# talmolab/track-mjx

Hardware: AMD Instinct MI355X
Metric: env-steps/sec (whole node), rodent task @ 4096 envs/GPU (higher is better)
Workload: dtype f32

## Files before the change

### track_mjx_amd/csrc/wave_physics.h

```cpp
#pragma once
#include "tm_common.h"
#include "wave_layout.h"

#ifdef TM_HOST_EMU
#define TMW_NL 64
#define TMW_FOR for (int lane = 0; lane < 64; lane++)
#define TMW_SYNC() do { } while (0)
#define TMW_LI lane
#define TMW_LANE_DECL
#else
#define TMW_NL 1
#define TMW_FOR if (true)
#ifdef TMW_HARD_SYNC
#define TMW_SYNC() __syncthreads()
#else
#define TMW_SYNC() do { __builtin_amdgcn_fence(__ATOMIC_RELEASE, "wavefront"); __builtin_amdgcn_wave_barrier(); __builtin_amdgcn_fence(__ATOMIC_ACQUIRE, "wavefront"); } while (0)
#endif
#define TMW_LI 0
#define TMW_LANE_DECL const int lane = c.lane;
#endif
#define TMW_REG(type, name) type name[TMW_NL]
#ifdef TM_HOST_EMU
#define TMW_DUP_LANES_OK 0
#else
#define TMW_DUP_LANES_OK 1
#endif
#define TMW_DS 7

#ifdef TM_HOST_EMU
typedef const DModel TmwModel;
#else
typedef const __attribute__((address_space(4))) DModel TmwModel;
#endif
#define TMW_LOCAL(name, n, src) float name[n]; { _Pragma("unroll") for (int k_ = 0; k_ < (n); k_++) name[k_] = (src)[k_]; }
#ifdef TMW_RAND
#define TMW_RAND_ONLY(...) __VA_ARGS__
#define TMW_SCALE(x, s) tmw_scaled((x), c.s)
#ifdef TM_HOST_EMU
TM_DEV float tmw_scaled(float x, float s) { volatile float r = x * s; return r; }
#else
TM_DEV float tmw_scaled(float x, float s) { float r = x * s; asm volatile("" : "+v"(r)); return r; }
#endif
TM_DEV float tmw_rand_invweight(float t, float mu, float impratio) {
  const float mm = tmw_scaled(mu, mu), a = tmw_scaled(mm, t), b = tmw_scaled(t + a, 2.f), d = tmw_scaled(b, mu), e = tmw_scaled(d, mu);
  return e / impratio;
}
#define TMW_CON_IW(cc) tmw_rand_invweight(m.con_tw[cc], TMW_MU(cc), m.impratio)
#else
#define TMW_RAND_ONLY(...)
#define TMW_SCALE(x, s) x
#define TMW_CON_IW(cc) m.con_invweight[cc]
#endif
#define TMW_EMU_HAS_QA 1
struct WCtx {
  TmwModel *mp;
  float *L;
  float *st;
  int n, e;
  int lane;
  unsigned long long *prof;
  unsigned long long tlast;
  float *dump;
  int nact;
  int nla;
  int rs;
  unsigned kmask[TMW_NL];
  const float *action;
  float qfs0[TMW_NL], qfs1[TMW_NL];
  float dg0[TMW_NL], dg1[TMW_NL];
  float wp0[TMW_NL], wp1[TMW_NL];
  float qa0[TMW_NL], qa1[TMW_NL];
  float ma0[TMW_NL], ma1[TMW_NL];
  int tp0[TMW_NL], tp1[TMW_NL];
  float *mspill;
  TMW_RAND_ONLY(float s_f, s_a, s_d;)
};
#define TMW_STATS(K) L[(K).l_com + 3]
#if defined(TMW_PROFILE) && !defined(TM_HOST_EMU)
#define TMW_TICK(idx) do { unsigned long long t_ = __builtin_amdgcn_s_memtime(); if (c.prof && c.lane == 0) c.prof[idx] += t_ - c.tlast; c.tlast = t_; } while (0)
#define TMW_TICK2(idx) TMW_TICK(idx)
#define TMW_COUNT(idx, v) do { if (c.prof && c.lane == 0) c.prof[idx] += (v); } while (0)
#else
#define TMW_TICK(idx) do { } while (0)
#define TMW_TICK2(idx) do { } while (0)
#define TMW_COUNT(idx, v) do { } while (0)
#endif
#define WST(off, i) c.st[c.rs ? (size_t)c.e * (size_t)c.rs + (size_t)((off) + (i)) : (size_t)((off) + (i)) * (size_t)c.n + (size_t)c.e]

#define TMW_ACT(a) (*(K.lean ? &WST(m.s_act, (a)) : &L[K.l_act + (a)]))
#define TMW_QFS(i) (K.lean ? ((i) < 64 ? c.qfs0[TMW_LI] : c.qfs1[TMW_LI]) : L[K.l_qfrc_smooth + (i)])
#define TMW_QFS_SET(i, v) do { if (!K.lean) L[K.l_qfrc_smooth + (i)] = (v); else if ((i) < 64) c.qfs0[TMW_LI] = (v); else c.qfs1[TMW_LI] = (v); } while (0)
#ifdef TMW_NO_QA_REGS
#define TMW_QAREG(K) 0
#else
#define TMW_QAREG(K) ((K).lean)
#endif
#define TMW_QA(i) (TMW_QAREG(K) ? ((i) < 64 ? c.qa0[TMW_LI] : c.qa1[TMW_LI]) : L[K.l_qacc + (i)])
#define TMW_QA_SET(i, v) do { if (!TMW_QAREG(K)) L[K.l_qacc + (i)] = (v); else if ((i) < 64) c.qa0[TMW_LI] = (v); else c.qa1[TMW_LI] = (v); } while (0)
#define TMW_MA(i) (TMW_QAREG(K) ? ((i) < 64 ? c.ma0[TMW_LI] : c.ma1[TMW_LI]) : L[K.l_Ma + (i)])
#define TMW_MA_SET(i, v) do { if (!TMW_QAREG(K)) L[K.l_Ma + (i)] = (v); else if ((i) < 64) c.ma0[TMW_LI] = (v); else c.ma1[TMW_LI] = (v); } while (0)
#define TMW_OK1(K) (lane + 64 < (K).nv)
#define TMW_I1(K) (TMW_OK1(K) ? lane + 64 : lane)
#define TMW_MA1(K, i1) (TMW_QAREG(K) ? c.ma1[TMW_LI] : L[(K).l_Ma + (i1)])
#define TMW_QA1(K, i1) (TMW_QAREG(K) ? c.qa1[TMW_LI] : L[(K).l_qacc + (i1)])
#define TMW_DG(i) ((i) < 64 ? c.dg0[TMW_LI] : c.dg1[TMW_LI])
#define TMW_WP(i) ((i) < 64 ? c.wp0[TMW_LI] : c.wp1[TMW_LI])
#define TMW_WP_SET(i, v) do { if ((i) < 64) c.wp0[TMW_LI] = (v); else c.wp1[TMW_LI] = (v); } while (0)
#define TMW_MU(cc) (K.lean ? TMW_SCALE(m.con_mu[0], s_f) : L[K.l_con_mu + (cc)])
#ifdef TMW_NO_EFCD_PACK
#define TMW_DIDX(kr) (kr)
#else
#define TMW_DIDX(kr) (K.lean ? ((kr) < c.nla ? (kr) : c.nla + (((kr) - c.nla) >> 2)) : (kr))
#endif
#define TMW_LIMSIGN(K) ((signed char *)(L + (K).l_lim_sign))
TM_DEV int tm_f2i(float f) { int i; __builtin_memcpy(&i, &f, 4); return i; }
TM_DEV float tm_i2f(int i) { float f; __builtin_memcpy(&f, &i, 4); return f; }

#ifdef TM_HOST_EMU
TM_DEV float tmw_sum(const float *v) { float s = 0.f; for (int i = 0; i < 64; i++) s += v[i]; return s; }
TM_DEV float tmw_readlane(const float *v, int src) { return v[src]; }
#else
template <int CTRL, int ROW_MASK, int BANK_MASK>
TM_DEV float tmw_dpp_add(float v) {
  int moved = __builtin_amdgcn_update_dpp(0, tm_f2i(v), CTRL, ROW_MASK, BANK_MASK, false);
  return v + tm_i2f(moved);
}
#ifdef TMW_SHFL_REDUCE
TM_DEV float tmw_sum(const float *vp) {
  float v = vp[0];
  for (int off = 32; off >= 1; off >>= 1) v += __shfl_xor(v, off);
  return v;
}
TM_DEV float tmw_readlane(const float *v, int src) { return __shfl(v[0], src); }
#define tmw_sum_dpp tmw_sum_unused
#define tmw_readlane_dpp tmw_readlane_unused
#else
#define tmw_sum_dpp tmw_sum
#define tmw_readlane_dpp tmw_readlane
#endif
TM_DEV float tmw_sum_dpp(const float *vp) {
  float v = vp[0];
  v = tmw_dpp_add<0x111, 0xf, 0xf>(v);
  v = tmw_dpp_add<0x112, 0xf, 0xf>(v);
  v = tmw_dpp_add<0x114, 0xf, 0xf>(v);
  v = tmw_dpp_add<0x118, 0xf, 0xf>(v);
  v = tmw_dpp_add<0x142, 0xf, 0xf>(v);
  v = tmw_dpp_add<0x143, 0xf, 0xf>(v);
  return tm_i2f(__builtin_amdgcn_readlane(tm_f2i(v), 63));
}
TM_DEV float tmw_readlane_dpp(const float *v, int src) { return tm_i2f(__builtin_amdgcn_readlane(tm_f2i(v[0]), src)); }
#endif
#ifdef TM_HOST_EMU
template <int WIDTH> TM_DEV float tmw_sum_w(const float *v) { return tmw_sum(v); }
#else
template <int WIDTH> TM_DEV float tmw_sum_w(const float *vp) {
  float v = vp[0];
  v = tmw_dpp_add<0x111, 0xf, 0xf>(v);
  v = tmw_dpp_add<0x112, 0xf, 0xf>(v);
  v = tmw_dpp_add<0x114, 0xf, 0xf>(v);
  v = tmw_dpp_add<0x118, 0xf, 0xf>(v);
  if (WIDTH <= 16) return tm_i2f(__builtin_amdgcn_readlane(tm_f2i(v), 15));
  v = tmw_dpp_add<0x142, 0xf, 0xf>(v);
  if (WIDTH <= 32) return tm_i2f(__builtin_amdgcn_readlane(tm_f2i(v), 31));
  v = tmw_dpp_add<0x143, 0xf, 0xf>(v);
  return tm_i2f(__builtin_amdgcn_readlane(tm_f2i(v), 63));
}
#endif
#ifdef TM_HOST_EMU
TM_DEV int tmw_table2(const float *a0, const float *a1, int idx) { return tm_f2i(idx < 64 ? a0[idx] : a1[idx - 64]); }
#else
TM_DEV int tmw_table2(const float *a0, const float *a1, int idx) { return __builtin_amdgcn_readlane(tm_f2i(idx < 64 ? a0[0] : a1[0]), idx & 63); }
#endif

#ifdef TM_HOST_EMU
TM_DEV int tmw_prefix(const int *flag, int *excl) { int s = 0; for (int l = 0; l < 64; l++) { excl[l] = s; s += flag[l] != 0; } return s; }
#else
TM_DEV int tmw_prefix(const int *flag, int *excl) {
  unsigned long long b = __builtin_amdgcn_ballot_w64(flag[0] != 0);
  excl[0] = (int)__builtin_amdgcn_mbcnt_hi((unsigned)(b >> 32), __builtin_amdgcn_mbcnt_lo((unsigned)b, 0u));
  return __builtin_popcountll(b);
}
#endif
#define TMW_ROWMAP(K) ((unsigned char *)(L + (K).l_rowmap))
#define TMW_CCROW(K) ((unsigned char *)(L + (K).l_ccrow))
#define TMW_CONGRP(K) ((unsigned char *)(L + (K).l_con_grpb) + (K).ncon)

TM_DEV float tmw_load_state(WCtx &c, const WLayout &K, const float *action) {
  TmwModel &m = *c.mp; float *L = c.L; TMW_LANE_DECL
  TMW_FOR { for (int i = lane; i < K.lds_floats; i += 64) L[i] = 0.f; }
  TMW_SYNC();
  TMW_FOR {
    for (int i = lane; i < K.nq + K.nv + (K.lean ? 0 : K.nu); i += 64) L[K.l_qpos + i] = WST(m.s_qpos, i);
    if (K.lean) {
      c.tp0[TMW_LI] = m.tpack[lane < K.nv ? lane : 0]; c.tp1[TMW_LI] = m.tpack[lane + 64 < K.nv ? lane + 64 : 64];
      for (int g = lane; g < K.ngroup; g += 64) L[K.l_tgrp + g] = tm_i2f(m.gpack[g]);
    } else {
      for (int i = lane; i < 2 * K.nv; i += 64) {
        int dof = i >> 1, extra = (i & 1) ? m.dof_wsub[dof] + 1 : m.dof_limrow[dof] + 1;
        L[K.l_tdof + i] = tm_i2f(m.tdof[i] | (extra << 24));
      }
      for (int g = lane; g < K.ngroup; g += 64) ((signed char *)(L + K.l_tgrp))[g] = (signed char)m.grp_lastdof[g];
    }
    for (int cc = lane; cc < K.ncon; cc += 64) { if (!K.lean) L[K.l_con_mu + cc] = TMW_SCALE(m.con_mu[cc], s_f); TMW_CONGRP(K)[cc] = (unsigned char)m.con_grp[cc]; }
    {
      int su = lane / 6;
      bool ok = lane < m.n_wsub * 6;
      c.kmask[TMW_LI] = ok ? m.wsub_cmask[su][0] : 0u;
    }
  }
  TMW_SYNC();
  return WST(m.s_time, 0);
}
#define TMW_MEND(w0) ((w0) & 0xffff)
#define TMW_DEPTH(w0) (((w0) >> 16) & 0xff)
#define TMW_ADR(w0) (((w0) & 0xffff) - TMW_DEPTH(w0))
#define TMW_LIMROW1(w0) (((w0) >> 24) & 0xff)
#define TMW_WSUB1(w1) (((w1) >> 24) & 0xff)
#define TMW_W0(i) tm_f2i(L[K.l_tdof + 2 * (i)])
#define TMW_W1(i) tm_f2i(L[K.l_tdof + 2 * (i) + 1])
TM_DEV int tmw_anc(int i, int q, int w1) {
  int r = i - (w1 & 0xff);
  return q <= r ? i - q : ((w1 >> 8) & 0xff) + r - q;
}
#ifdef TM_HOST_EMU
TM_DEV int tmw_opaque_v(int x) { return x; }
#else
TM_DEV int tmw_opaque_v(int x) { asm volatile("" : "+v"(x)); return x; }
#endif
#define TMW_TP(i) tmw_opaque_v((i) < 64 ? c.tp0[TMW_LI] : c.tp1[TMW_LI])
#define TMW_TP_MEND(p) ((p) & 0x7ff)
#define TMW_TP_DEPTH(p) (((p) >> 11) & 0x3f)
#define TMW_TP_RUN(p) (((p) >> 17) & 0x1f)
#define TMW_TP_WSUB1(p) (((p) >> 22) & 0xf)
TM_DEV int tmw_anc_r(int i, int q, int r, int jp1) { return q <= r ? i - q : jp1 + r - q; }
TM_DEV void tmw_store_state(WCtx &c, const WLayout &K, float time) {
  TmwModel &m = *c.mp; float *L = c.L; TMW_LANE_DECL
  TMW_FOR {
    for (int i = lane; i < K.nq + K.nv + (K.lean ? 0 : K.nu); i += 64) WST(m.s_qpos, i) = L[K.l_qpos + i];
    if (lane == 0) WST(m.s_time, 0) = time;
  }
  TMW_SYNC();
}

TM_DEV void tmw_put_con_frame(float *L, const WLayout &K, int cc, const float *fr) {
  if (K.lean) { if (cc == 0) for (int k = 0; k < 3; k++) L[K.l_con_frame + k] = fr[k]; for (int k = 0; k < 3; k++) L[K.l_con_frame + 3 + cc * 3 + k] = fr[3 + k]; }
  else for (int k = 0; k < 6; k++) L[K.l_con_frame + cc * 6 + k] = fr[k];
}
TM_DEV void tmw_get_con_frame(const float *L, const WLayout &K, int cc, float *fr) {
  if (K.lean) { for (int k = 0; k < 3; k++) { fr[k] = L[K.l_con_frame + k]; fr[3 + k] = L[K.l_con_frame + 3 + cc * 3 + k]; } }
  else for (int k = 0; k < 6; k++) fr[k] = L[K.l_con_frame + cc * 6 + k];
}

TM_DEV void tmw_position(WCtx &c, const WLayout &K, bool emit) {
  TmwModel &m = *c.mp; float *L = c.L; TMW_LANE_DECL
  const int HB = K.lean ? 4 : 0;
  TMW_FOR {
    float rec[2][16];
#pragma unroll
    for (int slot = 0; slot < (K.lean ? 1 : 2); slot++) {
      const int b = lane + HB + 64 * slot < K.nbody ? lane + HB + 64 * slot : K.nbody - 1;
#pragma unroll
      for (int k = 0; k < 16; k++) rec[slot][k] = m.body_kin[b][k];
    }
#pragma unroll
    for (int slot = 0; slot < (K.lean ? 1 : 2); slot++) {
      const int b = lane + HB + 64 * slot;
      if (b >= K.nbody) continue;
      const float *rc = rec[slot];
      float t[3] = {rc[0], rc[1], rc[2]};
      float q[4] = {rc[3], rc[4], rc[5], rc[6]};
      for (int jj = 0; jj < m.body_jntnum[b]; jj++) {
        int j = m.body_jntadr[b] + jj, qa, jtype;
        float jpos[3], jaxis[3], q0;
        if (jj == 0) {
          jtype = tm_f2i(rc[7]); qa = tm_f2i(rc[8]); q0 = rc[15];
          for (int k = 0; k < 3; k++) { jpos[k] = rc[9 + k]; jaxis[k] = rc[12 + k]; }
        } else {
          jtype = m.jnt_type[j]; qa = m.jnt_qposadr[j]; q0 = m.qpos0[qa];
          for (int k = 0; k < 3; k++) { jpos[k] = m.jnt_pos[j][k]; jaxis[k] = m.jnt_axis[j][k]; }
        }
        if (!K.lean && jtype == 0) {
          for (int k = 0; k < 3; k++) t[k] = L[K.l_qpos + qa + k];
          for (int k = 0; k < 4; k++) q[k] = L[K.l_qpos + qa + 3 + k];
          tm_normalize4(q);
          for (int k = 0; k < 4; k++) L[K.l_qpos + qa + 3 + k] = q[k];
          for (int k = 0; k < 3; k++) { L[K.l_jl_anchor + j * 3 + k] = t[k]; L[K.l_jl_axis + j * 3 + k] = (k == 2) ? 1.f : 0.f; }
        } else {
          float r[3], an[3], ax[3], ql[4], q2[4];
          tm_rotate(r, jpos, q);
          for (int k = 0; k < 3; k++) an[k] = t[k] + r[k];
          tm_rotate(ax, jaxis, q);
// ... 188 lines not shown
        tm_quat_to_mat(X, q);
        off[0] = (b < 64 ? xo0[TMW_LI] : xo3[TMW_LI]) - com[0]; off[1] = (b < 64 ? xo1[TMW_LI] : xo4[TMW_LI]) - com[1]; off[2] = (b < 64 ? xo2[TMW_LI] : xo5[TMW_LI]) - com[2];
        float oo = tm_dot3(off, off);
        ci[0] = X[0] * in[0] * X[0] + X[1] * in[1] * X[1] + X[2] * in[2] * X[2] + (oo - off[0] * off[0]) * mass;
        ci[1] = X[3] * in[0] * X[3] + X[4] * in[1] * X[4] + X[5] * in[2] * X[5] + (oo - off[1] * off[1]) * mass;
        ci[2] = X[6] * in[0] * X[6] + X[7] * in[1] * X[7] + X[8] * in[2] * X[8] + (oo - off[2] * off[2]) * mass;
        ci[3] = X[0] * in[0] * X[3] + X[1] * in[1] * X[4] + X[2] * in[2] * X[5] - off[0] * off[1] * mass;
        ci[4] = X[0] * in[0] * X[6] + X[1] * in[1] * X[7] + X[2] * in[2] * X[8] - off[0] * off[2] * mass;
        ci[5] = X[3] * in[0] * X[6] + X[4] * in[1] * X[7] + X[5] * in[2] * X[8] - off[1] * off[2] * mass;
        ci[6] = off[0] * mass; ci[7] = off[1] * mass; ci[8] = off[2] * mass; ci[9] = mass;
      }
      for (int k = 0; k < 10; k++) L[K.l_cinert + b * 10 + k] = ci[k];
    }
  }
  TMW_SYNC();
}

TM_DEV void tmw_chain_scan(WCtx &c, const WLayout &K, int base) {
  float *L = c.L; TMW_LANE_DECL
  TMW_FOR {
    if (lane < 6) {
      float *p = L + base + lane, v[TMW_RODENT_TRUNK], acc = 0.f;
#pragma unroll
      for (int t = 0; t < TMW_RODENT_TRUNK; t++) v[t] = p[t * TMW_DS];
#pragma unroll
      for (int t = 0; t < TMW_RODENT_TRUNK; t++) { acc += v[t]; p[t * TMW_DS] = acc; }
    }
  }
  TMW_SYNC();
  TMW_FOR {
    if (lane < TMW_RODENT_NCHAIN * 6) {
      const int ci = lane / 6, k = lane - ci * 6;
      int first = 0, n = 0, d0 = 1, idx = 0;
#define TMW_X(f, nn, dd) if (ci == idx) { first = f; n = nn; d0 = dd; } idx++;
      TMW_RODENT_LEAF_CHAINS(TMW_X)
#undef TMW_X
      float acc = L[base + (d0 - 1) * TMW_DS + k];
      float *p = L + base + first * TMW_DS + k;
      constexpr int MAXN = tmw_chain_maxrun(TMW_RODENT_TRUNK, 73) + 1, UB = 8;
      float keep = 0.f;
#pragma unroll 1
      for (int t0 = 0; t0 < MAXN; t0 += UB) {
        float v[UB];
#pragma unroll
        for (int u = 0; u < UB; u++) v[u] = p[(t0 + u < n ? t0 + u : n - 1) * TMW_DS];
#pragma unroll
        for (int u = 0; u < UB; u++) { acc += v[u]; keep = t0 + u < n ? acc : keep; p[(t0 + u < n ? t0 + u : n - 1) * TMW_DS] = keep; }
      }
    }
  }
  TMW_SYNC();
}

TM_DEV void tmw_velocity_inertia(WCtx &c, const WLayout &K) {
  TmwModel &m = *c.mp; float *L = c.L; TMW_LANE_DECL
  int R = K.nround_dof + (K.nround_dof & 1);
  TMW_FOR {
    const bool ok1 = TMW_OK1(K); const int i1 = TMW_I1(K);
    const float qv0 = L[K.l_qvel + lane], qv1 = L[K.l_qvel + i1];
    float cd0[6], cd1[6];
    for (int k = 0; k < 6; k++) { cd0[k] = L[K.l_cdof + lane * 6 + k]; cd1[k] = L[K.l_cdof + i1 * 6 + k]; }
    float *o0 = L + K.l_dscanA + lane * TMW_DS, *o1 = L + K.l_dscanA + i1 * TMW_DS;
    for (int k = 0; k < 6; k++) o0[k] = cd0[k] * qv0;
    if (!K.chains) o0[6] = tm_i2f(m.dof_parentid[lane]);
    if (ok1) { for (int k = 0; k < 6; k++) o1[k] = cd1[k] * qv1; if (!K.chains) o1[6] = tm_i2f(m.dof_parentid[i1]); }
  }
  TMW_SYNC();
  if (K.chains) tmw_chain_scan(c, K, K.l_dscanA);
  else
  for (int r = 0; r < R; r++) {
    const float *cur = L + ((r & 1) ? K.l_dscanB : K.l_dscanA);
    float *nxt = L + ((r & 1) ? K.l_dscanA : K.l_dscanB);
    TMW_FOR {
      for (int i = lane; i < K.nv; i += 64) {
        const float *s = cur + i * TMW_DS;
        float v[6] = {s[0], s[1], s[2], s[3], s[4], s[5]};
        int a = tm_f2i(s[6]);
        if (a >= 0) { const float *sa = cur + a * TMW_DS; for (int k = 0; k < 6; k++) v[k] += sa[k]; a = tm_f2i(sa[6]); }
        float *o = nxt + i * TMW_DS;
        for (int k = 0; k < 6; k++) o[k] = v[k];
        o[6] = tm_i2f(a);
      }
    }
    TMW_SYNC();
  }
  TMW_TICK2(20);
  float dd0[TMW_NL][6], dd1[TMW_NL][6], cv0[TMW_NL][6], cv1[TMW_NL][6];
  TMW_FOR {
    for (int slot = 0; slot < 2; slot++) {
      int i = lane + 64 * slot;
      float *dd = slot ? dd1[TMW_LI] : dd0[TMW_LI];
      for (int k = 0; k < 6; k++) dd[k] = 0.f;
      if (i < K.nv && !m.dof_freetrans[i]) {
        int vp = m.dof_vpar[i];
        float E[6] = {0.f, 0.f, 0.f, 0.f, 0.f, 0.f}, cd[6];
        if (vp >= 0) for (int k = 0; k < 6; k++) E[k] = L[K.l_dscanA + vp * TMW_DS + k];
        for (int k = 0; k < 6; k++) cd[k] = L[K.l_cdof + i * 6 + k];
        tm_motion_cross(dd, E, cd);
      }
      int b = lane + 64 * slot;
      float *cv = slot ? cv1[TMW_LI] : cv0[TMW_LI];
      for (int k = 0; k < 6; k++) cv[k] = 0.f;
      if (b < K.nbody) { int ld = m.body_lastdof[b]; if (ld >= 0) for (int k = 0; k < 6; k++) cv[k] = L[K.l_dscanA + ld * TMW_DS + k]; }
    }
  }
  TMW_SYNC();
  TMW_FOR {
// ... 31 lines not shown
    for (int slot = 0; slot < 2; slot++) {
      int b = lane + 64 * slot;
      if (b >= K.nbody) continue;
      const float *cv = slot ? cv1[TMW_LI] : cv0[TMW_LI];
      float ca[6] = {0.f, 0.f, 0.f, -m.gravity[0], -m.gravity[1], -m.gravity[2]}, I[10], f1[6], t[6], f2[6];
      int ld = m.body_lastdof[b];
      if (ld >= 0) for (int k = 0; k < 6; k++) ca[k] += L[K.l_dscanA + ld * TMW_DS + k];
      for (int k = 0; k < 10; k++) I[k] = L[K.l_cinert + b * 10 + k];
      tm_inert_mul(f1, I, ca);
      tm_inert_mul(t, I, cv);
      tm_motion_cross_force(f2, cv, t);
      for (int k = 0; k < 6; k++) L[K.l_cfrc + b * 6 + k] = (b == 0) ? 0.f : f1[k] + f2[k];
    }
  }
  TMW_SYNC();
  TMW_TICK2(22);
  TMW_REG(float, ns0); TMW_REG(float, ns1);
  TMW_FOR { ns0[TMW_LI] = tm_i2f(lane < K.nbody ? m.body_nsub[lane] : 1); ns1[TMW_LI] = tm_i2f(lane + 64 < K.nbody ? m.body_nsub[lane + 64] : 1); }
  TMW_FOR {
    const int comp = lane & 15;
    const int base = comp < 10 ? K.l_cinert + comp : K.l_cfrc + comp - 10, stride = comp < 10 ? 10 : 6;
    float run = 0.f;
    for (int b0 = K.nbody - 1; b0 >= 1; b0 -= 8) {
      float vb[8]; int nb[8];
#pragma unroll
      for (int u = 0; u < 8; u++) { int b = b0 - u > 0 ? b0 - u : 0; vb[u] = L[base + b * stride]; nb[u] = tmw_table2(ns0, ns1, b); }
#pragma unroll
      for (int u = 0; u < 8; u++) {
        int b = b0 - u > 0 ? b0 - u : 0;
        run = vb[u] + (nb[u] > 1 ? run : 0.f);
        if (TMW_DUP_LANES_OK || lane < 16) L[base + b * stride] = run;
      }
    }
  }
  TMW_SYNC();
  for (int f = 0; f < m.n_fix; f++) {
    int p = m.fix_p[f], r0 = m.fix_r0[f];
    TMW_FOR {
      const int comp = lane & 15;
      const int base = comp < 10 ? K.l_cinert + comp : K.l_cfrc + comp - 10, stride = comp < 10 ? 10 : 6;
      float delta = 0.f;
      for (int e = m.fix_adr[f]; e < m.fix_adr[f + 1]; e++) delta += L[base + m.fix_child[e] * stride];
      for (int b = r0 + (lane >> 4); b <= p; b += 4) L[base + b * stride] += delta;
    }
    TMW_SYNC();
  }
  const bool has_bias = m.has_bias != 0;
  if (has_bias) {
    TMW_FOR {
      for (int a = lane; a < K.nu; a += 64) {
        const int e0 = m.act_madr[a], e1 = m.act_madr[a + 1];
        float len = 0.f;
        for (int e = e0; e < e1; e++) len += m.act_mval[e] * L[K.l_qpos + m.act_mqpos[e]];
        const float act = K.lean ? WST(m.s_act, a) : L[K.l_act + a];
        L[K.l_sv + a] = TMW_SCALE(m.act_gain[a], s_a) * act + (TMW_SCALE(m.act_b0[a], s_a) + TMW_SCALE(m.act_b1[a], s_a) * len);
      }
    }
  } else if (K.lean) { TMW_FOR { for (int a = lane; a < K.nu; a += 64) L[K.l_sv + a] = WST(m.s_act, a); } }
  TMW_SYNC();
  TMW_TICK2(23);
  TMW_REG(float, bias0); TMW_REG(float, bias1);
  TMW_FOR {
    const int i1 = TMW_I1(K), b0 = m.dof_bodyid[lane], b1 = m.dof_bodyid[i1];
    float cd0[6], cd1[6], cf0[6], cf1[6], s0 = 0.f, s1 = 0.f;
    for (int k = 0; k < 6; k++) { cd0[k] = L[K.l_cdof + lane * 6 + k]; cd1[k] = L[K.l_cdof + i1 * 6 + k]; cf0[k] = L[K.l_cfrc + b0 * 6 + k]; cf1[k] = L[K.l_cfrc + b1 * 6 + k]; }
    for (int k = 0; k < 6; k++) s0 += cd0[k] * cf0[k];
    for (int k = 0; k < 6; k++) s1 += cd1[k] * cf1[k];
    bias0[TMW_LI] = s0; if (TMW_OK1(K)) bias1[TMW_LI] = s1;
  }
  TMW_SYNC();
  TMW_FOR {
    float dd[2][8];
#pragma unroll
    for (int slot = 0; slot < 2; slot++) {
      const int i = lane + 64 * slot < K.nv ? lane + 64 * slot : K.nv - 1;
#pragma unroll
      for (int k = 0; k < 8; k++) dd[slot][k] = m.dof_dyn[i][k];
      TMW_RAND_ONLY(dd[slot][2] = tmw_scaled(dd[slot][2], c.s_d);)
    }
#pragma unroll
    for (int slot = 0; slot < 2; slot++) {
      const int i = lane + 64 * slot;
      if (i >= K.nv) continue;
      const float *rc = dd[slot];
      const int b = tm_f2i(rc[0]);
      float I[10], cd[6], buf[6];
      for (int k = 0; k < 10; k++) I[k] = L[K.l_cinert + b * 10 + k];
      for (int k = 0; k < 6; k++) cd[k] = L[K.l_cdof + i * 6 + k];
      tm_inert_mul(buf, I, cd);
      int adr, d, run, jp1;
      if (K.lean) { const int tp = TMW_TP(i); d = TMW_TP_DEPTH(tp); adr = TMW_TP_MEND(tp) - d; run = TMW_TP_RUN(tp); jp1 = d - run; }
      else { const int w0 = TMW_W0(i), w1 = TMW_W1(i); adr = TMW_ADR(w0); d = TMW_DEPTH(w0); run = i - (w1 & 0xff); jp1 = (w1 >> 8) & 0xff; }
#pragma unroll 4
      for (int k = 0; k <= d; k++) {
        const float *cj = L + K.l_cdof + tmw_anc_r(i, k, run, jp1) * 6;
        float s = buf[0] * cj[0] + buf[1] * cj[1] + buf[2] * cj[2] + buf[3] * cj[3] + buf[4] * cj[4] + buf[5] * cj[5];
        if (k == 0) s += rc[1];
        L[K.l_M + adr + k] = s;
      }
      const float bias = i < 64 ? bias0[TMW_LI] : bias1[TMW_LI];
      float fa = 0.f;
      if (has_bias) { for (int e = tm_f2i(rc[6]); e < tm_f2i(rc[7]); e++) fa += m.dof_act_coef[e] * L[K.l_sv + m.dof_act_id[e]]; }
      else for (int e = tm_f2i(rc[6]); e < tm_f2i(rc[7]); e++) { int u = m.dof_act_id[e]; fa += m.dof_act_coef[e] * (TMW_SCALE(m.dof_act_gain[e], s_a) * L[(K.lean ? K.l_sv : K.l_act) + u]); }
      WST(m.s_qfrc_actuator, i) = fa;
      float f = -rc[2] * L[K.l_qvel + i] - bias + fa;
      if (rc[3] != 0.f) f += -rc[3] * (L[K.l_qpos + tm_f2i(rc[4])] - rc[5]);
      TMW_QFS_SET(i, f);
    }
  }
  TMW_SYNC();
}

TM_DEV void tmw_factor(WCtx &c, const WLayout &K, float hdamp, int rhs = -1) {
  TmwModel &m = *c.mp; float *L = c.L; TMW_LANE_DECL
  TMW_FOR {
    for (int i = lane; i < K.nnz; i += 64) L[K.l_LD + i] = L[K.l_M + i];
  }
  TMW_SYNC();
  if (hdamp != 0.f) {
    TMW_FOR { for (int i = lane; i < K.nv; i += 64) L[K.l_LD + m.dof_Madr[i]] += hdamp * TMW_SCALE(m.dof_damping[i], s_d); }
    TMW_SYNC();
  }
  TMW_REG(float, a0); TMW_REG(float, a1); TMW_REG(float, b0); TMW_REG(float, b1); TMW_REG(float, acc); TMW_REG(float, pr);
  for (int i = K.nv - 1; i >= 0; i--) {
    int w0 = TMW_W0(i), adr = TMW_ADR(w0), d = TMW_DEPTH(w0), nd = (TMW_W1(i) >> 16) & 0xff;
    TMW_FOR {
      float rsum = 0.f;
#pragma unroll
      for (int slot = 0; slot < 2; slot++) {
        int t = lane + 64 * slot;
        float a = 0.f; int base = K.l_LD;
        if (t < nd) {
          int kk = i + nd - t, wk = TMW_W0(kk);
          base = K.l_LD + TMW_MEND(wk) - d;
          a = L[base] * L[K.l_Dinv + kk];
          if (rhs >= 0) rsum += a * L[rhs + kk];
        }
        (slot ? a1 : a0)[TMW_LI] = a; (slot ? b1 : b0)[TMW_LI] = tm_i2f(base);
      }
      acc[TMW_LI] = (lane <= d) ? L[K.l_LD + adr + lane] : 0.f;
      pr[TMW_LI] = rsum;
    }
    TMW_TICK2(13);
    if (rhs >= 0 && nd > 0) { float s = tmw_sum(pr); TMW_FOR { if (lane == 0) L[rhs + i] -= s; } }
    for (int slot = 0; slot < 2; slot++) {
      const float *ar = slot ? a1 : a0, *br = slot ? b1 : b0;
      int cnt = nd - 64 * slot; if (cnt > 64) cnt = 64;
      for (int t0 = 0; t0 < cnt; t0 += 8) {
        float a[8]; int bb[8];
#pragma unroll
        for (int u = 0; u < 8; u++) {
          int t = t0 + u < 64 ? t0 + u : 63;
          a[u] = tmw_readlane(ar, t);
          bb[u] = tm_f2i(tmw_readlane(br, t));
        }
        TMW_FOR {
          float v[8];
// ... 1141 lines not shown
    for (int sl = 0; sl < TMW_LS_SLOTS; sl++) {
      if (sl > 0 && (w16 || 64 * sl >= c.nact)) {
        R.ja[TMW_LI][sl] = 1.f; R.jv[TMW_LI][sl] = 0.f; R.D[TMW_LI][sl] = 0.f; R.t0[TMW_LI][sl] = 0.f; R.t1[TMW_LI][sl] = 0.f; R.t2[TMW_LI][sl] = 0.f;
        continue;
      }
      int e = w16 ? (lane & 15) : lane + 64 * sl;
      bool ok = w16 ? (sl == 0 && lane < 48 && e < c.nact) : e < c.nact;
      float ja = ok ? L[K.l_Jaref + (ok ? e : 0)] : 1.f, jv = ok ? L[K.l_jv + (ok ? e : 0)] : 0.f, D = ok ? L[K.l_efc_D + (ok ? TMW_DIDX(e) : 0)] : 0.f;
      R.ja[TMW_LI][sl] = ja; R.jv[TMW_LI][sl] = jv; R.D[TMW_LI][sl] = D;
      R.t0[TMW_LI][sl] = 0.5f * ja * ja * D; R.t1[TMW_LI][sl] = jv * ja * D; R.t2[TMW_LI][sl] = 0.5f * jv * jv * D;
    }
  }
  TMW_TICK2(13);
  float ia;
  if (c.nact <= 16) ia = tmw_ls_core<16>(c, K, R, g0, g1, g2, gtol);
  else if (c.nact <= 32) ia = tmw_ls_core<32>(c, K, R, g0, g1, g2, gtol);
  else ia = tmw_ls_core<64>(c, K, R, g0, g1, g2, gtol);
  TMW_TICK2(14);
  TMW_REG(float, pc); TMW_REG(float, pg);
  TMW_FOR {
    float sc = 0.f, sg = 0.f;
    {
      const bool ok1 = TMW_OK1(K); const int i1 = TMW_I1(K);
      const float sq0 = L[K.l_search + lane], sq1 = L[K.l_search + i1], m0 = L[K.l_mv + lane], m1 = L[K.l_mv + i1];
      const float qa0 = TMW_QA(lane) + sq0 * ia, ut0 = TMW_MA(lane) + m0 * ia;
      const float qa1 = TMW_QA1(K, i1) + sq1 * ia, ut1 = TMW_MA1(K, i1) + m1 * ia;
      TMW_QA_SET(lane, qa0); TMW_MA_SET(lane, ut0);
      if (ok1) { TMW_QA_SET(lane + 64, qa1); TMW_MA_SET(lane + 64, ut1); }
      sg += c.dg0[TMW_LI] * ut0 * ut0;
      sg += (ok1 ? c.dg1[TMW_LI] * ut1 : 0.f) * ut1;
    }
#pragma unroll
    for (int sl = 0; sl < TMW_LS_SLOTS; sl++) {
      int e = lane + 64 * sl;
      if (e < c.nact) { float ja = R.ja[TMW_LI][sl] + R.jv[TMW_LI][sl] * ia; L[K.l_Jaref + e] = ja; if (ja < 0.f) sc += R.D[TMW_LI][sl] * ja * ja; }
    }
    pc[TMW_LI] = sc; pg[TMW_LI] = sg;
  }
  TMW_SYNC();
  gauss = 0.5f * tmw_sum(pg);
  return 0.5f * tmw_sum(pc) + gauss;
}
TM_DEV void tmw_solve_cg(WCtx &c, const WLayout &K) {
  TmwModel &m = *c.mp; float *L = c.L; TMW_LANE_DECL
  float gauss, scale = m.meaninertia * (float)(K.nv > 1 ? K.nv : 1);
#if defined(TMW_PROFILE) && !defined(TM_HOST_EMU)
  if (c.prof && c.lane == 0) { c.prof[10] += (c.nact <= 16) ? 1000 : 0; c.prof[18] += (c.nact > 16 && c.nact <= 32) ? 1000 : 0; }
#endif
  TMW_FOR {
    c.dg1[TMW_LI] = 0.f; c.wp1[TMW_LI] = 0.f;
    if (TMW_QAREG(K)) { c.qa1[TMW_LI] = 0.f; c.ma1[TMW_LI] = 0.f; }
    {
      const bool ok1 = TMW_OK1(K); const int i1 = TMW_I1(K);
      const float wq0 = WST(m.s_warm, lane), wq1 = WST(m.s_warm, i1);
      const float ma0 = L[K.l_Ma + lane], ma1 = L[K.l_Ma + i1], di0 = L[K.l_Dinv + lane], di1 = L[K.l_Dinv + i1];
      L[K.l_qacc + lane] = wq0;
      if (ok1) L[K.l_qacc + i1] = wq1;
      if (TMW_QAREG(K)) { c.qa0[TMW_LI] = wq0; c.ma0[TMW_LI] = ma0; if (ok1) { c.qa1[TMW_LI] = wq1; c.ma1[TMW_LI] = ma1; } }
      c.dg0[TMW_LI] = 1.f / di0; c.wp0[TMW_LI] = 0.f;
      if (ok1) { c.dg1[TMW_LI] = 1.f / di1; c.wp1[TMW_LI] = 0.f; }
    }
  }
  TMW_SYNC();
  float gs, cs = tmw_eval_cost(c, K, K.l_qacc_smooth, gs, true);
  float cw = tmw_eval_cost(c, K, K.l_qacc, gauss, false, K.m_spilled());
  float cost = cw;
  if (cw < cs) {
    TMW_FOR { for (int i = lane; i < K.nv; i += 64) L[K.l_Ma + i] -= TMW_QFS(i); }
    TMW_SYNC();
    tmw_solve_up(c, K, K.l_Ma, K.l_Ma);
    if (TMW_QAREG(K)) { TMW_FOR { for (int i = lane; i < K.nv; i += 64) TMW_MA_SET(i, L[K.l_Ma + i]); } }
  } else {
    TMW_FOR { for (int i = lane; i < K.nv; i += 64) { const float qs = L[K.l_qacc_smooth + i]; if (TMW_QAREG(K)) { TMW_QA_SET(i, qs); TMW_MA_SET(i, 0.f); } else { L[K.l_qacc + i] = qs; L[K.l_Ma + i] = 0.f; } } }
    TMW_SYNC();
    cost = tmw_eval_cost(c, K, TMW_QAREG(K) ? K.l_qacc_smooth : K.l_qacc, gauss, true);
  }
  float prev_cost = INFINITY, num;
  float gn = tmw_update_gradient(c, K, num);
  TMW_FOR { const int i1 = TMW_I1(K); const float g0 = L[K.l_Mgrad + lane], g1 = L[K.l_Mgrad + i1]; L[K.l_mv + lane] = -g0; if (TMW_OK1(K)) L[K.l_mv + i1] = -g1; }
  TMW_SYNC();
  TMW_TICK(6);
  TMW_STATS(K) = 0.f;
  int it = 0;
  for (; it < m.iterations; it++) {
    if (m.iterations != 1) {
      float improvement = (prev_cost - cost) / scale;
      float gradient = sqrtf(m.meaninertia * fmaxf(gn, 0.f)) / scale;
      if (improvement < m.tolerance || gradient < m.tolerance) break;
    }
    float cost_new = tmw_linesearch(c, K, gauss);
    TMW_TICK(7);
    TMW_COUNT(36, 1000);
    TMW_FOR { const float g0 = L[K.l_Mgrad + lane], g1 = L[K.l_Mgrad + TMW_I1(K)]; c.wp0[TMW_LI] = g0; if (TMW_OK1(K)) c.wp1[TMW_LI] = g1; }
    prev_cost = cost;
    cost = cost_new;
    float den = gn;
#ifndef TMW_CG_NO_EARLY_EXIT
    const float last_if = it + 1 >= m.iterations ? INFINITY : m.tolerance;
#else
    const float last_if = -INFINITY;
#endif
    gn = tmw_update_gradient(c, K, num, (prev_cost - cost) / scale, last_if);
    if (gn >= 0.f) {
      float beta = fmaxf(0.f, num / fmaxf(TM_MINVAL, den));
      TMW_FOR {
        const int i1 = TMW_I1(K);
        const float g0 = L[K.l_Mgrad + lane], g1 = L[K.l_Mgrad + i1], s0 = L[K.l_mv + lane], s1 = L[K.l_mv + i1];
        L[K.l_mv + lane] = -g0 + beta * s0; if (TMW_OK1(K)) L[K.l_mv + i1] = -g1 + beta * s1;
      }
      TMW_SYNC();
    }
    TMW_TICK(8);
  }
  TMW_STATS(K) += 64.f * (float)it;
  TMW_FOR { for (int i = lane; i < K.nv; i += 64) WST(m.s_warm, i) = TMW_QA(i); }
  if (c.dump) { TMW_FOR { for (int i = lane; i < K.nv; i += 64) c.dump[(size_t)(m.w_qacc + i) * (size_t)c.n + (size_t)c.e] = TMW_QA(i); } }
  if (c.dump) { TMW_FOR { for (int i = lane; i < K.nv; i += 64) c.dump[(size_t)(m.w_qfrc_constraint + i) * (size_t)c.n + (size_t)c.e] = L[K.l_qfrc_constraint + i]; } }
  TMW_SYNC();
}

TM_DEV void tmw_forward(WCtx &c, const WLayout &K, bool emit) {
  TmwModel &m = *c.mp; float *L = c.L; TMW_LANE_DECL
  TMW_TICK(12);
#ifndef TMW_STOP
#define TMW_STOP 99
#endif
  tmw_position(c, K, emit);
  TMW_TICK(0);
  if (TMW_STOP <= 0) return;
  tmw_velocity_inertia(c, K);
  TMW_TICK(1);
  if (TMW_STOP <= 1) return;
  if (K.m_spilled()) {
    TmwModel &m = *c.mp;
    TMW_REG(float, w0); TMW_REG(float, w1);
    TMW_FOR { w0[TMW_LI] = WST(m.s_warm, lane); w1[TMW_LI] = lane + 64 < K.nv ? WST(m.s_warm, lane + 64) : 0.f; }
    TMW_FOR {
      constexpr int NB = 6;
      for (int i0 = lane; i0 < K.nnz; i0 += 64 * NB) {
        float v[NB];
#pragma unroll
        for (int u = 0; u < NB; u++) { const int i = i0 + 64 * u; v[u] = L[K.l_M + (i < K.nnz ? i : K.nnz - 1)]; }
#pragma unroll
        for (int u = 0; u < NB; u++) { const int i = i0 + 64 * u; if (i < K.nnz) c.mspill[i] = v[u]; }
      }
    }
    TMW_FOR { L[K.l_qacc + lane] = w0[TMW_LI]; if (lane + 64 < K.nv) L[K.l_qacc + lane + 64] = w1[TMW_LI]; }
    TMW_SYNC();
    tmw_mul_m(c, K, K.l_qacc, K.l_Ma);
  }
  if (K.chains) tmw_factor_chains<false>(c, K, 0.f, -1); else tmw_factor(c, K, 0.f);
  TMW_TICK(2);
  if (TMW_STOP <= 2) return;
  if (K.chains) tmw_invert_chains(c, K); else tmw_invert_l(c, K);
  TMW_TICK(3);
  if (TMW_STOP <= 3) return;
  tmw_make_constraint(c, K);
  TMW_TICK(4);
  if (TMW_STOP <= 4) return;
  TMW_FOR { L[K.l_qacc_smooth + lane] = TMW_QFS(lane); if (TMW_OK1(K)) L[K.l_qacc_smooth + lane + 64] = TMW_QFS(lane + 64); }
  TMW_SYNC();
  tmw_solve(c, K, K.l_qacc_smooth, K.l_Mgrad);
  if (c.dump) { TMW_FOR { for (int i = lane; i < K.nv; i += 64) c.dump[(size_t)(m.w_qacc_smooth + i) * (size_t)c.n + (size_t)c.e] = L[K.l_qacc_smooth + i]; } }
  TMW_TICK(5);
  tmw_solve_cg(c, K);
}
TM_DEV float tmw_euler(WCtx &c, const WLayout &K, float time) {
  TmwModel &m = *c.mp; float *L = c.L; TMW_LANE_DECL
  float h = m.timestep;
  constexpr int MAXU = 20;
  float mr[TMW_NL][MAXU];
  if (K.m_spilled()) {
    TMW_FOR {
#pragma unroll
      for (int u = 0; u < MAXU; u++) { int i = lane + 64 * u; if (64 * u < K.nnz) mr[TMW_LI][u] = c.mspill[i < K.nnz ? i : K.nnz - 1]; }
    }
  }
  TMW_FOR { const int i1 = TMW_I1(K); const float f0 = L[K.l_qfrc_constraint + lane], f1 = L[K.l_qfrc_constraint + i1]; L[K.l_Mgrad + lane] = TMW_QFS(lane) + f0; if (TMW_OK1(K)) L[K.l_Mgrad + i1] = TMW_QFS(lane + 64) + f1; }
  TMW_FOR {
    { const int i1 = TMW_I1(K); const float dm0 = TMW_SCALE(m.dof_damping[lane], s_d), dm1 = TMW_SCALE(m.dof_damping[i1], s_d); L[K.l_hdamp + lane] = m.timestep * dm0; if (TMW_OK1(K)) L[K.l_hdamp + i1] = m.timestep * dm1; }
    for (int a = lane; a < K.nu; a += 64) {
      float ctrl = c.rs ? c.st[(size_t)c.e * (size_t)c.rs + (size_t)(m.s_prev_ctrl + a)] : (c.action ? c.action[(size_t)a * c.n + c.e] : 0.f);
      ctrl = fminf(fmaxf(ctrl, m.act_ctrlrange[a][0]), m.act_ctrlrange[a][1]);
      const float act = TMW_ACT(a);
      TMW_ACT(a) = act + ((ctrl - act) / fmaxf(TM_MINVAL, m.act_tau[a])) * h;
    }
  }
  if (K.m_spilled()) {
    TMW_FOR {
#pragma unroll
      for (int u = 0; u < MAXU; u++) { int i = lane + 64 * u; if (64 * u < K.nnz && i < K.nnz) L[K.l_M + i] = mr[TMW_LI][u]; }
    }
  }
  TMW_SYNC();
  TMW_TICK(8);
  if (K.chains) tmw_factor_chains<true>(c, K, h, K.l_Mgrad); else tmw_factor(c, K, h, K.l_Mgrad);
  TMW_TICK(9);
  if (K.chains) tmw_subst_chains(c, K, K.l_Mgrad); else tmw_subst_down(c, K, K.l_Mgrad);
  TMW_TICK(11);
  TMW_FOR {
    { const int i1 = TMW_I1(K); const float v0 = L[K.l_qvel + lane], v1 = L[K.l_qvel + i1], g0 = L[K.l_Mgrad + lane], g1 = L[K.l_Mgrad + i1]; L[K.l_qvel + lane] = v0 + g0 * h; if (TMW_OK1(K)) L[K.l_qvel + i1] = v1 + g1 * h; }
  }
  TMW_SYNC();
  TMW_FOR {
    for (int j = lane; j < K.njnt; j += 64) {
      int qa = m.jnt_qposadr[j], da = m.jnt_dofadr[j];
      if (m.jnt_type[j] == 0) {
        for (int k = 0; k < 3; k++) L[K.l_qpos + qa + k] += h * L[K.l_qvel + da + k];
        float v[3] = {L[K.l_qvel + da + 3], L[K.l_qvel + da + 4], L[K.l_qvel + da + 5]}, q[4], qr[4], q2[4];
        for (int k = 0; k < 4; k++) q[k] = L[K.l_qpos + qa + 3 + k];
        float nn = tm_normalize3(v), ang = h * nn * 0.5f, sn, cs;
        sincosf(ang, &sn, &cs);
        qr[0] = cs; qr[1] = v[0] * sn; qr[2] = v[1] * sn; qr[3] = v[2] * sn;
        tm_quat_mul(q2, q, qr);
        tm_normalize4(q2);
        for (int k = 0; k < 4; k++) L[K.l_qpos + qa + 3 + k] = q2[k];
      } else {
        L[K.l_qpos + qa] += h * L[K.l_qvel + da];
      }
    }
  }
  TMW_SYNC();
  return time + h;
}

TM_DEV void tmw_dump(WCtx &c, const WLayout &K, float *ws) {
  TmwModel &m = *c.mp; float *L = c.L; TMW_LANE_DECL
#define WDUMP(row, i) ws[(size_t)((row) + (i)) * (size_t)c.n + (size_t)c.e]
  TMW_FOR {
    for (int i = lane; i < K.nnz; i += 64) WDUMP(m.w_M, i) = K.m_spilled() ? c.mspill[i] : L[K.l_M + i];
    for (int i = lane; i < K.nv * 6; i += 64) WDUMP(m.w_cdof, i) = L[K.l_cdof + i];
    for (int i = lane; i < K.nv; i += 64) {
      WDUMP(m.w_qfrc_smooth, i) = TMW_QFS(i);
    }
    for (int i = lane; i < K.ncon; i += 64) WDUMP(m.w_con_dist, i) = L[K.l_con_dist + i];
    for (int cc = lane; cc < K.ncon; cc += 64) {
      float fr[9];
      tmw_get_con_frame(L, K, cc, fr);
      tm_cross(fr + 6, fr, fr + 3);
      for (int k = 0; k < 9; k++) WDUMP(m.w_con_frame, cc * 9 + k) = fr[k];
    }
    for (int r = lane; r < K.nefc; r += 64) {
      int kr = -1;
      if (r < K.nlim) { float sv = (float)TMW_LIMSIGN(K)[r]; if (sv != 0.f) kr = (int)fabsf(sv) - 1; }
// ... 225 lines not shown
```

Before: 1.704 million.

## Keep warm-start, activation and control state in registers across substeps

```diff
diff --git a/track_mjx_amd/csrc/wave_physics.h b/track_mjx_amd/csrc/wave_physics.h
--- a/track_mjx_amd/csrc/wave_physics.h
+++ b/track_mjx_amd/csrc/wave_physics.h
@@ -51,6 +51,7 @@
 #define TMW_SCALE(x, s) x
 #define TMW_CON_IW(cc) m.con_invweight[cc]
 #endif
+#define TMW_MAXU 20
 #define TMW_EMU_HAS_QA 1
 struct WCtx {
   TmwModel *mp;
@@ -74,6 +75,9 @@
   int tp0[TMW_NL], tp1[TMW_NL];
   float *mspill;
   TMW_RAND_ONLY(float s_f, s_a, s_d;)
+  float ws0[TMW_NL], ws1[TMW_NL];
+  float actr[TMW_NL];
+  float ctl[TMW_NL];
 };
 #define TMW_STATS(K) L[(K).l_com + 3]
 #if defined(TMW_PROFILE) && !defined(TM_HOST_EMU)
@@ -87,7 +91,12 @@
 #endif
 #define WST(off, i) c.st[c.rs ? (size_t)c.e * (size_t)c.rs + (size_t)((off) + (i)) : (size_t)((off) + (i)) * (size_t)c.n + (size_t)c.e]
 
-#define TMW_ACT(a) (*(K.lean ? &WST(m.s_act, (a)) : &L[K.l_act + (a)]))
+#define TMW_ACT(a) (K.lean ? c.actr[TMW_LI] : L[K.l_act + (a)])
+#define TMW_ACT_SET(a, v) do { if (K.lean) c.actr[TMW_LI] = (v); else L[K.l_act + (a)] = (v); } while (0)
+#define TMW_WARM(i) (K.lean ? ((i) < 64 ? c.ws0[TMW_LI] : c.ws1[TMW_LI]) : WST(m.s_warm, (i)))
+#define TMW_WARM_SET(i, v) do { if (!K.lean) WST(m.s_warm, (i)) = (v); else if ((i) < 64) c.ws0[TMW_LI] = (v); else c.ws1[TMW_LI] = (v); } while (0)
+#define TMW_CTRL_LOAD(a) fminf(fmaxf(c.rs ? c.st[(size_t)c.e * (size_t)c.rs + (size_t)(m.s_prev_ctrl + (a))] : (c.action ? c.action[(size_t)(a) * c.n + c.e] : 0.f), \
+                                     m.act_ctrlrange[a][0]), m.act_ctrlrange[a][1])
 #define TMW_QFS(i) (K.lean ? ((i) < 64 ? c.qfs0[TMW_LI] : c.qfs1[TMW_LI]) : L[K.l_qfrc_smooth + (i)])
 #define TMW_QFS_SET(i, v) do { if (!K.lean) L[K.l_qfrc_smooth + (i)] = (v); else if ((i) < 64) c.qfs0[TMW_LI] = (v); else c.qfs1[TMW_LI] = (v); } while (0)
 #ifdef TMW_NO_QA_REGS
@@ -192,6 +201,11 @@
   TMW_FOR {
     for (int i = lane; i < K.nq + K.nv + (K.lean ? 0 : K.nu); i += 64) L[K.l_qpos + i] = WST(m.s_qpos, i);
     if (K.lean) {
+      c.ws0[TMW_LI] = WST(m.s_warm, lane); c.ws1[TMW_LI] = TMW_OK1(K) ? WST(m.s_warm, lane + 64) : 0.f;
+      const int a = lane < K.nu ? lane : 0;
+      c.actr[TMW_LI] = WST(m.s_act, a); c.ctl[TMW_LI] = TMW_CTRL_LOAD(a);
+    }
+    if (K.lean) {
       c.tp0[TMW_LI] = m.tpack[lane < K.nv ? lane : 0]; c.tp1[TMW_LI] = m.tpack[lane + 64 < K.nv ? lane + 64 : 64];
       for (int g = lane; g < K.ngroup; g += 64) L[K.l_tgrp + g] = tm_i2f(m.gpack[g]);
     } else {
@@ -237,6 +251,10 @@
   TmwModel &m = *c.mp; float *L = c.L; TMW_LANE_DECL
   TMW_FOR {
     for (int i = lane; i < K.nq + K.nv + (K.lean ? 0 : K.nu); i += 64) WST(m.s_qpos, i) = L[K.l_qpos + i];
+    if (K.lean) {
+      for (int a = lane; a < K.nu; a += 64) WST(m.s_act, a) = c.actr[TMW_LI];
+      for (int i = lane; i < K.nv; i += 64) WST(m.s_warm, i) = TMW_WARM(i);
+    }
     if (lane == 0) WST(m.s_time, 0) = time;
   }
   TMW_SYNC();
@@ -531,7 +549,7 @@
   TMW_SYNC();
 }
 
-TM_DEV void tmw_velocity_inertia(WCtx &c, const WLayout &K) {
+TM_DEV void tmw_velocity_inertia(WCtx &c, const WLayout &K, bool emit) {
   TmwModel &m = *c.mp; float *L = c.L; TMW_LANE_DECL
   int R = K.nround_dof + (K.nround_dof & 1);
   TMW_FOR {
@@ -669,11 +687,11 @@
         const int e0 = m.act_madr[a], e1 = m.act_madr[a + 1];
         float len = 0.f;
         for (int e = e0; e < e1; e++) len += m.act_mval[e] * L[K.l_qpos + m.act_mqpos[e]];
-        const float act = K.lean ? WST(m.s_act, a) : L[K.l_act + a];
+        const float act = TMW_ACT(a);
         L[K.l_sv + a] = TMW_SCALE(m.act_gain[a], s_a) * act + (TMW_SCALE(m.act_b0[a], s_a) + TMW_SCALE(m.act_b1[a], s_a) * len);
       }
     }
-  } else if (K.lean) { TMW_FOR { for (int a = lane; a < K.nu; a += 64) L[K.l_sv + a] = WST(m.s_act, a); } }
+  } else if (K.lean) { TMW_FOR { for (int a = lane; a < K.nu; a += 64) L[K.l_sv + a] = TMW_ACT(a); } }
   TMW_SYNC();
   TMW_TICK2(23);
   TMW_REG(float, bias0); TMW_REG(float, bias1);
@@ -719,7 +737,7 @@
       float fa = 0.f;
       if (has_bias) { for (int e = tm_f2i(rc[6]); e < tm_f2i(rc[7]); e++) fa += m.dof_act_coef[e] * L[K.l_sv + m.dof_act_id[e]]; }
       else for (int e = tm_f2i(rc[6]); e < tm_f2i(rc[7]); e++) { int u = m.dof_act_id[e]; fa += m.dof_act_coef[e] * (TMW_SCALE(m.dof_act_gain[e], s_a) * L[(K.lean ? K.l_sv : K.l_act) + u]); }
-      WST(m.s_qfrc_actuator, i) = fa;
+      if (emit || c.dump) WST(m.s_qfrc_actuator, i) = fa;
       float f = -rc[2] * L[K.l_qvel + i] - bias + fa;
       if (rc[3] != 0.f) f += -rc[3] * (L[K.l_qpos + tm_f2i(rc[4])] - rc[5]);
       TMW_QFS_SET(i, f);
@@ -1967,7 +1985,7 @@
     if (TMW_QAREG(K)) { c.qa1[TMW_LI] = 0.f; c.ma1[TMW_LI] = 0.f; }
     {
       const bool ok1 = TMW_OK1(K); const int i1 = TMW_I1(K);
-      const float wq0 = WST(m.s_warm, lane), wq1 = WST(m.s_warm, i1);
+      const float wq0 = K.lean ? c.ws0[TMW_LI] : WST(m.s_warm, lane), wq1 = K.lean ? c.ws1[TMW_LI] : WST(m.s_warm, i1);
       const float ma0 = L[K.l_Ma + lane], ma1 = L[K.l_Ma + i1], di0 = L[K.l_Dinv + lane], di1 = L[K.l_Dinv + i1];
       L[K.l_qacc + lane] = wq0;
       if (ok1) L[K.l_qacc + i1] = wq1;
@@ -2028,7 +2046,7 @@
     TMW_TICK(8);
   }
   TMW_STATS(K) += 64.f * (float)it;
-  TMW_FOR { for (int i = lane; i < K.nv; i += 64) WST(m.s_warm, i) = TMW_QA(i); }
+  TMW_FOR { for (int i = lane; i < K.nv; i += 64) TMW_WARM_SET(i, TMW_QA(i)); }
   if (c.dump) { TMW_FOR { for (int i = lane; i < K.nv; i += 64) c.dump[(size_t)(m.w_qacc + i) * (size_t)c.n + (size_t)c.e] = TMW_QA(i); } }
   if (c.dump) { TMW_FOR { for (int i = lane; i < K.nv; i += 64) c.dump[(size_t)(m.w_qfrc_constraint + i) * (size_t)c.n + (size_t)c.e] = L[K.l_qfrc_constraint + i]; } }
   TMW_SYNC();
@@ -2043,13 +2061,10 @@
   tmw_position(c, K, emit);
   TMW_TICK(0);
   if (TMW_STOP <= 0) return;
-  tmw_velocity_inertia(c, K);
+  tmw_velocity_inertia(c, K, emit);
   TMW_TICK(1);
   if (TMW_STOP <= 1) return;
   if (K.m_spilled()) {
-    TmwModel &m = *c.mp;
-    TMW_REG(float, w0); TMW_REG(float, w1);
-    TMW_FOR { w0[TMW_LI] = WST(m.s_warm, lane); w1[TMW_LI] = lane + 64 < K.nv ? WST(m.s_warm, lane + 64) : 0.f; }
     TMW_FOR {
       constexpr int NB = 6;
       for (int i0 = lane; i0 < K.nnz; i0 += 64 * NB) {
@@ -2060,7 +2075,10 @@
         for (int u = 0; u < NB; u++) { const int i = i0 + 64 * u; if (i < K.nnz) c.mspill[i] = v[u]; }
       }
     }
-    TMW_FOR { L[K.l_qacc + lane] = w0[TMW_LI]; if (lane + 64 < K.nv) L[K.l_qacc + lane + 64] = w1[TMW_LI]; }
+    TMW_FOR {
+      const float w0 = K.lean ? c.ws0[TMW_LI] : WST(m.s_warm, lane), w1 = K.lean ? c.ws1[TMW_LI] : (TMW_OK1(K) ? WST(m.s_warm, lane + 64) : 0.f);
+      L[K.l_qacc + lane] = w0; if (TMW_OK1(K)) L[K.l_qacc + lane + 64] = w1;
+    }
     TMW_SYNC();
     tmw_mul_m(c, K, K.l_qacc, K.l_Ma);
   }
@@ -2083,28 +2101,26 @@
 TM_DEV float tmw_euler(WCtx &c, const WLayout &K, float time) {
   TmwModel &m = *c.mp; float *L = c.L; TMW_LANE_DECL
   float h = m.timestep;
-  constexpr int MAXU = 20;
-  float mr[TMW_NL][MAXU];
+  float mr[TMW_NL][TMW_MAXU];
   if (K.m_spilled()) {
     TMW_FOR {
 #pragma unroll
-      for (int u = 0; u < MAXU; u++) { int i = lane + 64 * u; if (64 * u < K.nnz) mr[TMW_LI][u] = c.mspill[i < K.nnz ? i : K.nnz - 1]; }
+      for (int u = 0; u < TMW_MAXU; u++) { int i = lane + 64 * u; if (64 * u < K.nnz) mr[TMW_LI][u] = c.mspill[i < K.nnz ? i : K.nnz - 1]; }
     }
   }
   TMW_FOR { const int i1 = TMW_I1(K); const float f0 = L[K.l_qfrc_constraint + lane], f1 = L[K.l_qfrc_constraint + i1]; L[K.l_Mgrad + lane] = TMW_QFS(lane) + f0; if (TMW_OK1(K)) L[K.l_Mgrad + i1] = TMW_QFS(lane + 64) + f1; }
   TMW_FOR {
     { const int i1 = TMW_I1(K); const float dm0 = TMW_SCALE(m.dof_damping[lane], s_d), dm1 = TMW_SCALE(m.dof_damping[i1], s_d); L[K.l_hdamp + lane] = m.timestep * dm0; if (TMW_OK1(K)) L[K.l_hdamp + i1] = m.timestep * dm1; }
     for (int a = lane; a < K.nu; a += 64) {
-      float ctrl = c.rs ? c.st[(size_t)c.e * (size_t)c.rs + (size_t)(m.s_prev_ctrl + a)] : (c.action ? c.action[(size_t)a * c.n + c.e] : 0.f);
-      ctrl = fminf(fmaxf(ctrl, m.act_ctrlrange[a][0]), m.act_ctrlrange[a][1]);
+      const float ctrl = K.lean ? c.ctl[TMW_LI] : TMW_CTRL_LOAD(a);
       const float act = TMW_ACT(a);
-      TMW_ACT(a) = act + ((ctrl - act) / fmaxf(TM_MINVAL, m.act_tau[a])) * h;
+      TMW_ACT_SET(a, act + ((ctrl - act) / fmaxf(TM_MINVAL, m.act_tau[a])) * h);
     }
   }
   if (K.m_spilled()) {
     TMW_FOR {
 #pragma unroll
-      for (int u = 0; u < MAXU; u++) { int i = lane + 64 * u; if (64 * u < K.nnz && i < K.nnz) L[K.l_M + i] = mr[TMW_LI][u]; }
+      for (int u = 0; u < TMW_MAXU; u++) { int i = lane + 64 * u; if (64 * u < K.nnz && i < K.nnz) L[K.l_M + i] = mr[TMW_LI][u]; }
     }
   }
   TMW_SYNC();
```

After: 1.713 million, median of 6. About the same (+0.5%).
